# dmytroleonenko/gym-narde

Measured on AMD Instinct MI355X. Metric: env steps/sec at batch=65536, 1 MI355X (+ legal-move bit-exact vs CPU), higher is better.
Workload: dtype u32

## Files before the change

### __graft_entry__.py

```python
import os
import subprocess
import sys

ROOT = os.path.dirname(os.path.abspath(__file__))
PKG_DIR = os.path.join(ROOT, "gym-narde_amd")
CSRC = os.path.join(PKG_DIR, "csrc")
LIB = os.path.join(PKG_DIR, "gym_narde", "libnarde.so")
HOSTCHECK = os.path.join(ROOT, "tests", "hostcheck")

HIPCC = os.environ.get("HIPCC", "/opt/rocm/bin/hipcc")
HIP_FLAGS = ["-O3", "-std=c++17", "--offload-arch=gfx950", "-fPIC", "-shared", "-Wall"]


def _paths():
    for p in (PKG_DIR, os.path.join(ROOT, "oracle")):
        if p not in sys.path:
            sys.path.insert(0, p)


def _run(cmd):
    print("+", " ".join(cmd), flush=True)
    subprocess.check_call(cmd)


def build():
    srcs = [os.path.join(CSRC, "narde.hip"), os.path.join(CSRC, "dqn_learner.hip")]
    _run([HIPCC, *HIP_FLAGS, "-o", LIB, *srcs])
    _run(["make", "-s", "-C", os.path.join(ROOT, "oracle")])
    os.makedirs(os.path.join(HOSTCHECK, "build"), exist_ok=True)
    _run([HIPCC, "-O2", "-std=c++17", "-fPIC", "-shared", "-x", "c++", "-D__HIP_PLATFORM_AMD__",
          "-I/opt/rocm/include", "-o", os.path.join(HOSTCHECK, "build", "libhostcheck.so"),
          os.path.join(HOSTCHECK, "hostcheck.cpp")])
    _run([HIPCC, "-O2", "-std=c++17", "-fPIC", "-shared", "-x", "c++", "-D__HIP_PLATFORM_AMD__",
          "-I/opt/rocm/include", "-o", os.path.join(HOSTCHECK, "build", "libhostcheck_afterstates.so"),
          os.path.join(HOSTCHECK, "hostcheck_afterstates.cpp")])
    _run([HIPCC, "-O2", "-std=c++17", "-fPIC", "-shared", "-x", "c++", "-D__HIP_PLATFORM_AMD__",
          "-I/opt/rocm/include", "-o", os.path.join(HOSTCHECK, "build", "libhostcheck_turn_afterstates.so"),
          os.path.join(HOSTCHECK, "hostcheck_turn_afterstates.cpp")])
    _run([HIPCC, "-O2", "-std=c++17", "-fPIC", "-shared", "-x", "c++", "-D__HIP_PLATFORM_AMD__",
          "-I/opt/rocm/include", "-o", os.path.join(HOSTCHECK, "build", "libhostcheck_value.so"),
          os.path.join(HOSTCHECK, "hostcheck_value.cpp")])
    _paths()
    import gym_narde
    import gym_narde.envs
    import gym_narde.vector
    from gym_narde import _lib

    _lib.load()


def smoke():
    _paths()
    import numpy as np
    import torch

    import oracle as O
    from gym_narde.envs.narde import Narde
    from gym_narde.vector import VecNardeEnv

    assert torch.cuda.is_available(), "smoke() needs a GPU"
    n, plies, seed = 2048, 64, 20251015
    env = VecNardeEnv(n, device="cuda:0", seed=seed, env_id_offset=5, max_episode_steps=1000)
    ref = O.SelfPlay(n, seed=seed, env0=5)
    ref.reset(0)
    rec = ref.run(plies)
    for p in range(plies):
        obs, rew, term, trunc, info = env.step()
        torch.cuda.synchronize()
        assert np.array_equal(obs.cpu().numpy(), rec["obs"][p].astype(np.int32)), f"obs ply {p}"
        assert np.array_equal(rew.cpu().numpy(), rec["reward"][p].astype(np.int32)), f"reward ply {p}"
        assert np.array_equal(term.cpu().numpy(), rec["terminated"][p]), f"terminated ply {p}"
        assert np.array_equal(info["actions"].cpu().numpy(), rec["action"][p]), f"actions ply {p}"
        assert np.array_equal(info["legal"].cpu().numpy().view(np.uint64), rec["legal"][p]), f"legal ply {p}"
    st = env.get_state()
    assert np.array_equal(st["board"].cpu().numpy(), ref.board)
    g = Narde()
    assert g.get_valid_moves([5, 3], 1) == [(23, 18)]
    assert g.get_valid_moves([6, 6], 1) == [(23, 17), (23, 17)]
    env.close()
    print(f"smoke ok: {n} envs x {plies} plies bit-exact vs oracle")


if __name__ == "__main__":
    build()
    if len(sys.argv) > 1 and sys.argv[1] == "smoke":
        smoke()
```

### gym-narde_amd/csrc/full4_wave.h

```cpp
#pragma once

namespace {

__device__ __forceinline__ uint32_t rl(uint32_t v, int l) {
  return (uint32_t)__builtin_amdgcn_readlane((int)v, l);
}
__device__ void coop_run(const Side& s, uint32_t low, int a, int b, int hl, uint32_t m0, uint32_t m1,
                         int need, bool bf, int mode, int lane, uint32_t out[3]) {
  out[0] = out[1] = out[2] = 0u;
  uint64_t owners = __ballot((m0 | m1) != 0u);
  const int which = lane >> 5, p = lane & 31;
  while (owners) {
    const int ow = (int)__builtin_ctzll(owners);
    owners &= owners - 1ull;
    Side c;
    c.own.w[0] = rl(s.own.w[0], ow); c.own.w[1] = rl(s.own.w[1], ow); c.own.w[2] = rl(s.own.w[2], ow);
    c.O = rl(s.O, ow); c.S1o = rl(s.S1o, ow); c.P = rl(s.P, ow);
    c.off_own = rl(s.off_own, ow);
    c.opp.w[0] = c.opp.w[1] = c.opp.w[2] = 0u;
    c.S1p = 0u; c.off_opp = 0u; c.ft_own = 0u; c.ft_opp = 0u; c.black = 0u; c.elapsed = 0u; c.t = 0u;
    const uint32_t lw = rl(low, ow), om0 = rl(m0, ow), om1 = rl(m1, ow);
    const int pa = (int)rl((uint32_t)a, ow), pb = (int)rl((uint32_t)b, ow);
    const int thl = (int)rl((uint32_t)hl, ow), tneed = (int)rl((uint32_t)need, ow);
    const bool tbf = rl(bf ? 1u : 0u, ow) != 0u;
// ... 148 lines not shown
  } else {
    Cl = 0u;
    if (xbf) { Ch = Lh; M = Lh ? Mx : 0; }
    else if (fast) { Ch = Lh; M = 4; }
    else if (!Lh) { Ch = 0u; M = 0; }
    else if (r0[2]) { Ch = r0[2]; M = 4; }
    else if (r0[1]) { Ch = r0[1]; M = 3; }
    else if (r0[0]) { Ch = r0[0]; M = 2; }
    else { Ch = Lh; M = 1; }
  }
  turn_play(s, dh, dl, Ch, Cl, M, hl0, play, pw, w, o,
            [&](int k, int dk, int need, bool act, int hl, uint32_t Lk) -> uint32_t {
              (void)k;
              if (act && !bf) Lk = die_filter(s.O, s.S1o, block_info_low(s.O, low), Lk, dk);
              if (hl <= 0) Lk &= ~HEAD;
              const bool direct = !dbl || bf || fast || need <= 0;
              uint32_t rk[3];
              coop_run(s, low, dk, 0, hl, (act && !direct) ? Lk : 0u, 0u, need > 0 ? need : 1, bf, 0, lane,
                       rk);
              return direct ? Lk : (need >= 2 ? rk[1] : rk[0]);
            });
}


__device__ void coop_depth_w(const Side& s, uint32_t fw, int d, int hl, uint32_t m0, int need, int lane,
                             uint32_t out[3]) {
  out[0] = out[1] = out[2] = 0u;
  uint64_t owners = __ballot(m0 != 0u);
  while (owners) {
    const int ow = (int)__builtin_ctzll(owners);
    owners &= owners - 1ull;
    Side c;
    c.own.w[0] = rl(s.own.w[0], ow); c.own.w[1] = rl(s.own.w[1], ow); c.own.w[2] = rl(s.own.w[2], ow);
    c.O = rl(s.O, ow); c.S1o = rl(s.S1o, ow); c.P = rl(s.P, ow);
    c.off_own = rl(s.off_own, ow);
    c.opp.w[0] = c.opp.w[1] = c.opp.w[2] = 0u;
    c.S1p = 0u; c.off_opp = 0u; c.ft_own = 0u; c.ft_opp = 0u; c.black = 0u; c.elapsed = 0u; c.t = 0u;
    const uint32_t ofw = rl(fw, ow), om = rl(m0, ow);
    const int od = (int)rl((uint32_t)d, ow), ohl = (int)rl((uint32_t)hl, ow), oneed = (int)rl((uint32_t)need, ow);
    const bool has = lane < 24 && ((om >> lane) & 1u);
    const int src = has ? lane : 0;
    Side cc = c;
    apply_die_if(cc, src, od, has);
    const int hl2 = ohl - ((has && src == 23) ? 1 : 0);
    int dep = oneed == 1 ? f4_probe_w<1>(cc, ofw, od, hl2)
                         : (oneed == 2 ? f4_probe_w<2>(cc, ofw, od, hl2) : f4_probe_w<3>(cc, ofw, od, hl2));
    const bool miss = has && dep < oneed;
    if (__ballot(miss) != 0ull) {
      if (miss)
        dep = oneed == 1 ? f4_depth_w<1>(cc, ofw, od, hl2)
                         : (oneed == 2 ? f4_depth_w<2>(cc, ofw, od, hl2) : f4_depth_w<3>(cc, ofw, od, hl2));
    }
    const bool k0 = has && dep >= 1, k1 = has && dep >= 2, k2 = has && dep >= 3;
    const uint32_t r0 = (uint32_t)__ballot(k0), r1 = (uint32_t)__ballot(k1), r2 = (uint32_t)__ballot(k2);
    out[0] = lane == ow ? r0 : out[0];
    out[1] = lane == ow ? r1 : out[1];
    out[2] = lane == ow ? r2 : out[2];
  }
}

__device__ void coop_pair_w(const Side& s, uint32_t fw, int d, int hl, uint32_t m0, uint32_t w0, int lane,
                            uint32_t r0[3], uint32_t& c1, bool& ok) {
  r0[0] = r0[1] = r0[2] = 0u;
  c1 = 0u;
  ok = false;
  uint64_t owners = __ballot(m0 != 0u);
  while (owners) {
    const int ow = (int)__builtin_ctzll(owners);
    owners &= owners - 1ull;
    Side c;
    c.own.w[0] = rl(s.own.w[0], ow); c.own.w[1] = rl(s.own.w[1], ow); c.own.w[2] = rl(s.own.w[2], ow);
    c.O = rl(s.O, ow); c.S1o = rl(s.S1o, ow); c.P = rl(s.P, ow);
    c.off_own = rl(s.off_own, ow);
    c.opp.w[0] = c.opp.w[1] = c.opp.w[2] = 0u;
    c.S1p = 0u; c.off_opp = 0u; c.ft_own = 0u; c.ft_opp = 0u; c.black = 0u; c.elapsed = 0u; c.t = 0u;
    const uint32_t ofw = rl(fw, ow), om = rl(m0, ow), ow0 = rl(w0, ow);
    const int od = (int)rl((uint32_t)d, ow), ohl = (int)rl((uint32_t)hl, ow);
    const int nsrc = __builtin_popcount(om);
    const int r = lane >> 3, k = lane & 7;
    const bool hs = r < nsrc;
    const int s0 = select_bit(om, hs ? r : 0);
    Side ca = c;
    apply_die_if(ca, s0, od, hs);
    const int hla = ohl - ((hs && s0 == 23) ? 1 : 0);
    uint32_t L1 = die_candidates_sl(ca.O, ca.P, od);
    L1 &= ~block_reject_w(ca.O, ca.S1o, ofw, L1, od);
    L1 &= hla <= 0 ? ~HEAD : ~0u;
    L1 = hs ? L1 : 0u;
    const int cnt = __builtin_popcount(L1);
    if (nsrc > 8 || __ballot(k == 0 && cnt > 8) != 0ull) continue;
    const bool hp = k < cnt;
    const int s1 = select_bit(L1, hp ? k : 0);
    Side cp = ca;
    apply_die_if(cp, s1, od, hp);
    const int hlp = hla - ((hp && s1 == 23) ? 1 : 0);
    int dep = f4_probe_w<2>(cp, ofw, od, hlp);
    const bool miss = hp && dep == 1;
    if (__ballot(miss) != 0ull) {
      if (miss) dep = f4_depth_w<2>(cp, ofw, od, hlp);
    }
    const uint64_t B0 = __ballot(k == 0 && cnt > 0), B1 = __ballot(hp && dep >= 1), B2 = __ballot(hp && dep >= 2);
    const bool src = lane < 24 && ((om >> lane) & 1u);
    const int rt = __builtin_popcount(om & ((1u << (lane & 31)) - 1u));
    const int sh = src ? 8 * rt : 0;
    const uint32_t a0 = (uint32_t)__ballot(src && ((B0 >> sh) & 1ull) != 0ull);
    const uint32_t a1 = (uint32_t)__ballot(src && ((B1 >> sh) & 0xFFull) != 0ull);
    const uint32_t a2 = (uint32_t)__ballot(src && ((B2 >> sh) & 0xFFull) != 0ull);
    const int M = a2 ? 4 : (a1 ? 3 : (a0 ? 2 : 1));
    const uint32_t Cs = a2 ? a2 : (a1 ? a1 : (a0 ? a0 : om));
    const int p0 = select_bit(Cs, (int)mulhi_u32(ow0, (uint32_t)__builtin_popcount(Cs)));
    const int r0p = __builtin_popcount(om & ((1u << p0) - 1u));
    const uint32_t Lp = rl(L1, 8 * r0p);
    const uint32_t G = (uint32_t)(((M >= 4 ? B2 : B1) >> (8 * r0p)) & 0xFFull);
    const bool inl = lane < 24 && ((Lp >> lane) & 1u);
    const int e = __builtin_popcount(Lp & ((1u << (lane & 31)) - 1u));
    const uint32_t cv = (uint32_t)__ballot(inl && ((G >> e) & 1u));
    r0[0] = lane == ow ? a0 : r0[0];
    r0[1] = lane == ow ? a1 : r0[1];
    r0[2] = lane == ow ? a2 : r0[2];
    c1 = lane == ow ? cv : c1;
    ok = lane == ow ? true : ok;
  }
}

__device__ __forceinline__ void ply_bound_turn_c0(Side& s, int dh, int dl, uint32_t bs, uint32_t fw,
                                                  const uint32_t w[4], bool flip_always, TurnOut& o, int lane,
                                                  const TurnC0& c) {
  uint32_t Lh = c.Lh, Ll = c.Ll, Ch = c.Ch, Cl = c.Cl;
  int M = c.M;
  const int hl0 = c.hl0;
  const bool dbl = dh == dl;
  const bool b2 = bs != 0u && !dbl, bd = bs != 0u && dbl;
  if (__ballot(b2) != 0ull) {
    if (b2) turn_c0_pair_bound_w(s, dh, dl, bs, fw, Lh, Ll, Ch, Cl, M);
  }
  bool srch = false, pairs = false;
  uint32_t c1p = 0u;
  if (__ballot(bd) != 0ull) {
    const uint32_t Lb = Lh & ~block_reject_w(s.O, s.S1o, bd ? fw : 0u, Lh, dh);
    const bool fast = bd && f4_safe_bound(s, dh, hl0, bs) >= 4;
    srch = bd && !fast && Lb != 0u;
    uint32_t r0[3];
    coop_pair_w(s, fw, dh, hl0, srch ? Lb : 0u, w[0], lane, r0, c1p, pairs);
    if (__ballot(srch && !pairs) != 0ull) {
      uint32_t rd[3];
      coop_depth_w(s, fw, dh, hl0, (srch && !pairs) ? Lb : 0u, 3, lane, rd);
      if (srch && !pairs) { r0[0] = rd[0]; r0[1] = rd[1]; r0[2] = rd[2]; }
    }
    const int Ms = r0[2] ? 4 : (r0[1] ? 3 : (r0[0] ? 2 : 1));
    const uint32_t Cs = r0[2] ? r0[2] : (r0[1] ? r0[1] : (r0[0] ? r0[0] : Lb));
    Ch = bd ? (fast ? Lb : (Lb ? Cs : 0u)) : Ch;
    M = bd ? (fast ? 4 : (Lb ? Ms : 0)) : M;
  }
  o.legal = (uint64_t)Ch | ((uint64_t)Cl << 24) | ((uint64_t)dh << 48) | ((uint64_t)dl << 52) |
            ((uint64_t)M << 56);
  const int nh = __builtin_popcount(Ch), n = nh + __builtin_popcount(Cl);
  const int idx = (int)mulhi_u32(w[0], (uint32_t)n);
  const bool hi = idx < nh;
  const int d0 = hi ? dh : dl;
  const int p0 = select_bit(hi ? Ch : Cl, hi ? idx : idx - nh);
  const bool go = M >= 1;
  apply_die_if(s, p0, d0, go);
  uint32_t pl0 = go ? (0xFFFF0000u | ((uint32_t)d0 << 8) | (uint32_t)p0) : 0xFFFFFFFFu, pl1 = 0xFFFFFFFFu;
  int hl = hl0 - ((go && p0 == 23) ? 1 : 0);
  const int d1 = dbl ? dh : (d0 == dh ? dl : dh);
  const bool anyb = __ballot(bs != 0u) != 0ull;
#pragma unroll
  for (int k = 1; k < 4; ++k) {
    const int dk = k == 1 ? d1 : dh;
    const bool act = k < M;
    uint32_t Lk = die_candidates_sl(s.O, s.P, dk);
    if (anyb) {
      const bool filt = bd || (k == 1 && b2);
      Lk &= ~block_reject_w(s.O, s.S1o, filt ? fw : 0u, Lk, dk);
    }
    Lk &= hl <= 0 ? ~HEAD : ~0u;
    const int need = M - k - 1;
    const bool byp = k == 1 && pairs && need > 0;
    Lk = (srch && act && byp) ? c1p : Lk;
    const bool chk = srch && act && need > 0 && !byp;
    if (__ballot(chk) != 0ull) {
      uint32_t rk[3];
      coop_depth_w(s, fw, dk, hl, chk ? Lk : 0u, need, lane, rk);
      Lk = chk ? (need >= 2 ? rk[1] : rk[0]) : Lk;
    }
    const uint32_t wk = k == 1 ? w[1] : (k == 2 ? w[2] : w[3]);
    const int p = select_bit(Lk, (int)mulhi_u32(wk, (uint32_t)__builtin_popcount(Lk)));
    apply_die_if(s, p, dk, act);
    const uint32_t v = ((uint32_t)dk << 8) | (uint32_t)p;
    if (k == 1) pl0 = act ? ((pl0 & 0xFFFFu) | (v << 16)) : pl0;
    if (k == 2) pl1 = act ? ((pl1 & 0xFFFF0000u) | v) : pl1;
    if (k == 3) pl1 = act ? ((pl1 & 0xFFFFu) | (v << 16)) : pl1;
    hl -= (act && p == 23) ? 1 : 0;
  }
  o.played = (uint64_t)pl0 | ((uint64_t)pl1 << 32);
  o.max_dice = M;
  o.term = s.off_own == 15u;
  o.reward = o.term ? (s.off_opp > 0u ? 1 : 2) : 0;
  if (flip_always) side_flip(s);
  else side_flip_if(s, !o.term);
}

__device__ __forceinline__ void ply_bound_turn(Side& s, int dh, int dl, uint32_t bs, uint32_t fw, const uint32_t w[4],
                                               bool flip_always, TurnOut& o, int lane) {
  TurnC0 c;
  turn_c0_free(s, dh, dl, c.Lh, c.Ll, c.Ch, c.Cl, c.M, c.hl0);
  ply_bound_turn_c0(s, dh, dl, bs, fw, w, flip_always, o, lane, c);
}

}
```

### gym-narde_amd/csrc/kernels_rollout.h

```cpp
#pragma once

namespace {

struct Outs {
  int32_t* __restrict__ obs;
  int32_t* __restrict__ reward;
  uint8_t* __restrict__ term;
  uint8_t* __restrict__ trunc;
  uint64_t* __restrict__ legal;
  int16_t* __restrict__ act_out;
  uint64_t* __restrict__ played;
  int64_t* __restrict__ totals;
};

struct StepArgs {
  Planes pl;
  int n;
  Rng g;
  int max_steps;
  int autoreset;
  const int16_t* __restrict__ actions;
  const int8_t* __restrict__ play;
  const uint8_t* __restrict__ dice;
  Outs out;
};

template <class T>
__device__ __forceinline__ void st_nt(T* p, T v) {
  if constexpr (sizeof(T) == 16) {
    typedef int v4nt __attribute__((ext_vector_type(4)));
    v4nt x;
    __builtin_memcpy(&x, &v, 16);
    __builtin_nontemporal_store(x, reinterpret_cast<v4nt*>(p));
  } else {
    __builtin_nontemporal_store(v, p);
  }
}

__device__ __forceinline__ int nib_at(uint32_t x, int off) {
  return (int)__builtin_amdgcn_ubfe(x, (uint32_t)off, 4u);
}

template <int B>
__device__ __forceinline__ int sub_byte(uint32_t a, uint32_t b) {
  int r;
  if constexpr (B == 0)
    asm("v_sub_u32_sdwa %0, %1, %2 dst_sel:DWORD dst_unused:UNUSED_PAD src0_sel:BYTE_0 src1_sel:BYTE_0"
        : "=v"(r) : "v"(a), "v"(b));
  else if constexpr (B == 1)
    asm("v_sub_u32_sdwa %0, %1, %2 dst_sel:DWORD dst_unused:UNUSED_PAD src0_sel:BYTE_1 src1_sel:BYTE_1"
        : "=v"(r) : "v"(a), "v"(b));
  else if constexpr (B == 2)
    asm("v_sub_u32_sdwa %0, %1, %2 dst_sel:DWORD dst_unused:UNUSED_PAD src0_sel:BYTE_2 src1_sel:BYTE_2"
        : "=v"(r) : "v"(a), "v"(b));
  else
    asm("v_sub_u32_sdwa %0, %1, %2 dst_sel:DWORD dst_unused:UNUSED_PAD src0_sel:BYTE_3 src1_sel:BYTE_3"
        : "=v"(r) : "v"(a), "v"(b));
  return r;
}

template <int Q>
__device__ __forceinline__ int4 obs_quad_w(uint32_t own, uint32_t opp) {
  const uint32_t ol = own & 0x0F0F0F0Fu, oh = (own >> 4) & 0x0F0F0F0Fu;
  const uint32_t pl = opp & 0x0F0F0F0Fu, ph = (opp >> 4) & 0x0F0F0F0Fu;
  if constexpr ((Q & 1) == 0)
    return make_int4(sub_byte<0>(ol, pl), sub_byte<0>(oh, ph), sub_byte<1>(ol, pl), sub_byte<1>(oh, ph));
  else
    return make_int4(sub_byte<2>(ol, pl), sub_byte<2>(oh, ph), sub_byte<3>(ol, pl), sub_byte<3>(oh, ph));
}

template <int Q>
__device__ __forceinline__ int4 obs_quad(const Side& s) {
  return obs_quad_w<Q>(s.own.w[Q >> 1], s.opp.w[Q >> 1]);
}

__device__ __forceinline__ void store_obs(int32_t* __restrict__ obs, size_t ix, const Side& s) {
  int4* o = reinterpret_cast<int4*>(obs + ix * 24);
  st_nt(o + 0, obs_quad<0>(s));
  st_nt(o + 1, obs_quad<1>(s));
  st_nt(o + 2, obs_quad<2>(s));
  st_nt(o + 3, obs_quad<3>(s));
  st_nt(o + 4, obs_quad<4>(s));
  st_nt(o + 5, obs_quad<5>(s));
}

__device__ __forceinline__ void store_obs_wave(int32_t* __restrict__ obs, size_t ix, const Side& s,
                                               int4* __restrict__ lds) {
  const int lane = threadIdx.x & 63;
  lds[lane * 6 + 0] = obs_quad<0>(s);
  lds[lane * 6 + 1] = obs_quad<1>(s);
  lds[lane * 6 + 2] = obs_quad<2>(s);
  lds[lane * 6 + 3] = obs_quad<3>(s);
  lds[lane * 6 + 4] = obs_quad<4>(s);
  lds[lane * 6 + 5] = obs_quad<5>(s);
  wave_lds_handoff();
  int4* dst = reinterpret_cast<int4*>(obs + (ix - lane) * 24);
#pragma unroll
  for (int q = 0; q < 6; ++q) st_nt(dst + q * 64 + lane, lds[q * 64 + lane]);
  wave_lds_handoff();
}

__device__ __forceinline__ void store_common(const Outs& out, size_t ix, const Side& s, int reward,
                                             int term, int trunc, int4* lds, bool via_lds) {
  if (out.obs) {
    if (via_lds) store_obs_wave(out.obs, ix, s, lds);
    else store_obs(out.obs, ix, s);
  }
  if (out.reward) st_nt(out.reward + ix, (int32_t)reward);
  if (out.term) st_nt(out.term + ix, (uint8_t)term);
  if (out.trunc) st_nt(out.trunc + ix, (uint8_t)trunc);
}

__device__ __forceinline__ void store_outs(const Outs& out, size_t ix, const Side& s,
                                           const StepOut& o, int term, int trunc, int4* lds,
                                           bool wave_full) {
  store_common(out, ix, s, o.reward, term, trunc, lds, wave_full);
  if (out.legal) st_nt(out.legal + ix, (uint64_t)compact_legal(o.l1));
  if (out.act_out)
    st_nt(reinterpret_cast<uint32_t*>(out.act_out) + ix,
           ((uint32_t)(uint16_t)o.code1) | ((uint32_t)(uint16_t)o.code2 << 16));
}

__device__ __forceinline__ void store_outs(const Outs& out, size_t ix, const Side& s,
                                           const TurnOut& o, int term, int trunc, int4* lds,
                                           bool wave_full) {
  (void)wave_full;
  store_common(out, ix, s, o.reward, term, trunc, lds, false);
  if (out.legal) st_nt(out.legal + ix, o.legal);
  if (out.played) st_nt(out.played + ix, o.played);
}

#define OBS_LDS_DECL                                   \
  __shared__ int4 obs_lds[kBlock * 6];                 \
  int4* const wave_lds = obs_lds + (threadIdx.x & ~63) * 6;

__device__ __forceinline__ void ply_draw_cached(const Rng& g, uint32_t t, uint32_t i, uint32_t R[4], bool first,
                                                uint32_t r[4]) {
  if (first || (t & 1u) == 0u) ply_block(t, g.env0 + i, g.k0, g.k1, R);
  ply_words_of(R, t, g.dice_mode, r);
}

__device__ __forceinline__ void ply(Side& s, int4& st, const Rng& g, uint32_t i,
                                    const int16_t* actions, const uint8_t* dice, int max_steps,
                                    bool autoreset, StepOut& o, int& term, int& trunc, uint32_t R[4],
                                    bool first) {
  uint32_t r[4];
  ply_draw_cached(g, s.t, i, R, first, r);
  int d0 = 0, d1 = 0, c1 = 0, c2 = 0;
  if (dice) { d0 = dice[2 * i]; d1 = dice[2 * i + 1]; }
  if (actions) { c1 = actions[2 * i]; c2 = actions[2 * i + 1]; }
  if (!dice && !actions && autoreset) env_ply_policy_sl(s, st, r, g.dice_mode, max_steps, o, term, trunc);
  else env_ply(s, st, r, dice != nullptr, d0, d1, g.dice_mode, actions == nullptr, c1, c2, max_steps,
               autoreset, o, term, trunc);
}

__device__ __forceinline__ void ply_draw_wave(const Rng& g, uint32_t t, uint32_t i, uint32_t R[4], int p, int par,
                                              uint32_t r[4]) {
  if (par >= 0) {
    if (p == 0 || ((par + p) & 1) == 0) ply_block(t, g.env0 + i, g.k0, g.k1, R);
  } else if (p == 0 || (t & 1u) == 0u) {
    ply_block(t, g.env0 + i, g.k0, g.k1, R);
  }
  ply_words_of(R, t, g.dice_mode, r);
}

__device__ __forceinline__ int wave_parity(bool valid, uint32_t t) {
  const uint64_t odd = __ballot(valid && (t & 1u)), vm = __ballot(valid);
  return odd == 0ull ? 0 : (odd == vm ? 1 : -1);
}

template <bool kFilt>
__device__ __forceinline__ void ply_free_turn(Side& s, int dh, int dl, uint32_t bs, uint32_t fw, const uint32_t w[4],
                                              bool flip_always, TurnOut& o, const TurnC0& c) {
  uint32_t Lh = c.Lh, Ll = c.Ll, Ch = c.Ch, Cl = c.Cl;
  int M = c.M;
  const bool b2 = kFilt && bs != 0u;
  if (kFilt && b2) turn_c0_pair_bound_w(s, dh, dl, bs, fw, Lh, Ll, Ch, Cl, M);
  turn_moves_sl(s, dh, dl, Ch, Cl, M, c.hl0, w, b2, fw, flip_always, o);
}

__device__ __forceinline__ void ply_full_turn(Side& s, int4& st, int dh, int dl, uint32_t bs, uint32_t fw,
                                              const TurnC0& c, const uint32_t w[4], uint32_t rb, int max_steps,
                                              bool autoreset, TurnOut& o, int& term, int& trunc) {
  const uint32_t mover_black = s.black;
  if (__ballot(bs != 0u && dh == dl) == 0ull) {
    if (__ballot(bs != 0u) == 0ull) ply_free_turn<false>(s, dh, dl, bs, fw, w, autoreset, o, c);
    else ply_free_turn<true>(s, dh, dl, bs, fw, w, autoreset, o, c);
  } else {
    ply_bound_turn_c0(s, dh, dl, bs, fw, w, autoreset, o, (int)(threadIdx.x & 63), c);
  }
  if (autoreset) ply_close_sl_b(s, st, o.term, o.reward, mover_black, rb, max_steps, term, trunc);
  else ply_close(s, st, o.term, o.reward, mover_black, 0u, max_steps, false, term, trunc);
}

__device__ __forceinline__ void ply_full_dice(Side& s, int4& st, int dh, int dl, const uint32_t w[4], uint32_t rb,
                                              int max_steps, bool autoreset, TurnOut& o, int& term, int& trunc) {
  const uint32_t low = block_lowmask(s.P);
  uint32_t fw;
  const uint32_t bs = turn_block_set_sl(s.O, s.S1o, s.P, low, dh, dl, fw);
  TurnC0 c;
  turn_c0_free(s, dh, dl, c.Lh, c.Ll, c.Ch, c.Cl, c.M, c.hl0);
  ply_full_turn(s, st, dh, dl, bs, fw, c, w, rb, max_steps, autoreset, o, term, trunc);
}

__device__ __forceinline__ uint32_t ply_dice_word(const uint32_t r[4], int dice_mode, uint32_t w[4]) {
  int d0, d1;
  dice_from(r[0], dice_mode, d0, d1);
  const int dh = d0 > d1 ? d0 : d1, dl = d0 > d1 ? d1 : d0;
  turn_words(r, w);
  return (uint32_t)dh | ((uint32_t)dl << 4) | (reset_black(r[3]) << 8);
}

__device__ __forceinline__ void ply_full_words(Side& s, int4& st, const uint32_t r[4], int dice_mode,
                                               int max_steps, bool autoreset, TurnOut& o, int& term,
                                               int& trunc) {
  uint32_t w[4];
  const uint32_t dw = ply_dice_word(r, dice_mode, w);
  ply_full_dice(s, st, (int)(dw & 15u), (int)((dw >> 4) & 15u), w, autoreset ? dw >> 8 : 0u, max_steps, autoreset,
                o, term, trunc);
}

__device__ __forceinline__ void ply_policy_full(Side& s, int4& st, const Rng& g, uint32_t i, int max_steps,
                                                bool autoreset, TurnOut& o, int& term, int& trunc,
                                                uint32_t R[4], int p, int par) {
  uint32_t r[4];
  ply_draw_wave(g, s.t, i, R, p, par, r);
  ply_full_words(s, st, r, g.dice_mode, max_steps, autoreset, o, term, trunc);
}

__device__ __forceinline__ void ply(Side& s, int4& st, const Rng& g, uint32_t i, bool valid,
                                    const int8_t* play, const uint8_t* dice, int max_steps,
                                    bool autoreset, TurnOut& o, int& term, int& trunc, uint32_t R[4],
                                    bool first) {
  if (!play && !dice) {
    ply_policy_full(s, st, g, i, max_steps, autoreset, o, term, trunc, R, 0, 0);
    return;
  }
  uint32_t r[4];
  ply_draw_cached(g, s.t, i, R, first, r);
  int d0 = 1, d1 = 2;
  if (dice && valid) { d0 = dice[2 * i]; d1 = dice[2 * i + 1]; }
  const uint64_t pw = (play && valid) ? reinterpret_cast<const uint64_t*>(play)[i] : ~0ull;
  const int lane = (int)(threadIdx.x & 63);
  env_ply_full_with(s, st, r, g.env0 + i, g.k0, g.k1, dice != nullptr, d0, d1, g.dice_mode,
                    play != nullptr, pw, max_steps, autoreset, o, term, trunc,
                    [&](Side& s2, int a, int b, bool pl, uint64_t pw2, const uint32_t* w2, TurnOut& o2) {
                      coop_turn_full(s2, a, b, pl, pw2, w2, o2, lane);
                    });
}

__device__ __forceinline__ void add_stats(int4* __restrict__ stats, int i, const int4& st) {
  if (st.x) {
    int4 cur = stats[i];
    cur.x += st.x; cur.y += st.y; cur.z += st.z;
    stats[i] = cur;
  }
}

__device__ __forceinline__ int4 stats_after(int4* __restrict__ stats, int i, const int4& st, bool want) {
  int4 cur = make_int4(0, 0, 0, 0);
  if (st.x || want) {
    cur = stats[i];
    cur.x += st.x; cur.y += st.y; cur.z += st.z;
    if (st.x) stats[i] = cur;
  }
  return cur;
}

__device__ __forceinline__ int4 stats_read(const int4* __restrict__ stats, int i, bool valid) {
  return valid ? stats[i] : make_int4(0, 0, 0, 0);
}
__device__ __forceinline__ int4 stats_after_pre(int4* __restrict__ stats, int i, int4 pre, const int4& st) {
  pre.x += st.x;
  pre.y += st.y;
  pre.z += st.z;
  if (st.x) stats[i] = pre;
  return pre;
}

__device__ __forceinline__ void wg_totals(const int4& cum, int64_t* __restrict__ rows) {
  __shared__ long long red[16][3];
  long long e = cum.x, w = cum.y, k = cum.z;
#pragma unroll
  for (int o = 32; o > 0; o >>= 1) {
    e += __shfl_xor(e, o, 64);
    w += __shfl_xor(w, o, 64);
    k += __shfl_xor(k, o, 64);
  }
  const int wave = threadIdx.x >> 6;
  if ((threadIdx.x & 63) == 0) { red[wave][0] = e; red[wave][1] = w; red[wave][2] = k; }
  __syncthreads();
  if (threadIdx.x < 3) {
    long long t = 0;
    const int nw = (int)(blockDim.x >> 6);
    for (int q = 0; q < nw; ++q) t += red[q][threadIdx.x];
    rows[3 * blockIdx.x + threadIdx.x] = (int64_t)t;
  }
}

template <bool kFull>
__global__ void __launch_bounds__(kBlock) k_step(StepArgs a) {
  OBS_LDS_DECL
  const int i = blockIdx.x * kBlock + threadIdx.x;
  const bool valid = i < a.n;
  if (!kFull && !valid) return;
  Side s = valid ? side_from_record(a.pl.p0[i], a.pl.p1[i]) : side_start(0u);
  int4 st = make_int4(0, 0, 0, 0);
  typename std::conditional<kFull, TurnOut, StepOut>::type o;
  int term, trunc;
  uint32_t R[4];
  if constexpr (kFull)
    ply(s, st, a.g, (uint32_t)i, valid, a.play, a.dice, a.max_steps, a.autoreset != 0, o, term, trunc, R,
        true);
  else
    ply(s, st, a.g, (uint32_t)i, a.actions, a.dice, a.max_steps, a.autoreset != 0, o, term, trunc, R, true);
  if (!valid) return;
  uint4 ra, rb;
  side_to_record(s, ra, rb);
  a.pl.p0[i] = ra;
  a.pl.p1[i] = rb;
  add_stats(a.pl.stats, i, st);
  store_outs(a.out, (size_t)i, s, o, term, trunc, wave_lds, i - (int)(threadIdx.x & 63) + 64 <= a.n);
}

constexpr int kPcGroups = 4;
constexpr int kPcEnvs = 64 * kPcGroups;
constexpr int kPcThreads = 2 * kPcEnvs;
constexpr int kPcR = 4;
constexpr int kPcSlots = 2;

__device__ __forceinline__ int pc_nblocks(int plies, int R) {
  return plies <= 1 ? 1 : 1 + (plies - 1 + R - 1) / R;
}
__device__ __forceinline__ void pc_block(int b, int plies, int R, int& p0, int& np) {
  p0 = b == 0 ? 0 : 1 + (b - 1) * R;
  const int sz = b == 0 ? 1 : R;
  np = max(0, min(sz, plies - p0));
}
constexpr int kPcRShort = 2;
constexpr int kPcShortPlies = 32;

struct PcLds {
  uint4 lead_[4];
  uint2 draw[kPcSlots][kPcR][kPcEnvs];
  uint4 nib0[kPcSlots][kPcR][kPcEnvs];
  uint2 nib1[kPcSlots][kPcR][kPcEnvs];
  uint2 legal[kPcSlots][kPcR][kPcEnvs];
  uint2 cf[kPcSlots][kPcR][kPcEnvs];
};

__device__ __forceinline__ void pc_put(PcLds& L, int slot, int k, int le, const Side& s,
                                       const StepOut& o, int term, int trunc) {
  const uint64_t lg = compact_legal(o.l1);
  L.nib0[slot][k][le] = make_uint4(s.own.w[0], s.own.w[1], s.own.w[2], s.opp.w[0]);
// ... 302 lines not shown
```

### gym-narde_amd/csrc/narde_rules.h

```cpp
#pragma once
#include <hip/hip_runtime.h>
#include <math.h>
#include <stdint.h>

#define NARDE_FN __host__ __device__ __forceinline__

namespace narde {

constexpr uint32_t MASK24 = 0xFFFFFFu;
constexpr int OFF = 24;

struct Nib {
  uint32_t w[3];
};

NARDE_FN uint32_t funnel16(uint32_t hi, uint32_t lo) { return (lo >> 16) | (hi << 16); }

NARDE_FN uint32_t nib_word(const Nib& b, int p) {
  const uint32_t w0 = b.w[0], w1 = b.w[1], w2 = b.w[2];
  const int k = p >> 3;
  return (k == 0 ? w0 : 0u) | (k == 1 ? w1 : 0u) | (k == 2 ? w2 : 0u);
}
NARDE_FN uint32_t nib_get(const Nib& b, int p) { return (nib_word(b, p) >> (4 * (p & 7))) & 15u; }
NARDE_FN void nib_add(Nib& b, int p, uint32_t delta ) {
// ... 1107 lines not shown
  const int tq = t > 0 ? t : 0;
  const uint32_t cf = nib_get(s.own, p);
  const bool land = en && !off;
  const uint32_t bf = en ? (1u << p) : 0u;
  const uint32_t bt = land ? (1u << tq) : 0u;
  const uint32_t vf = en ? (0xFFFFFFFFu << (4 * (p & 7))) : 0u;
  const uint32_t vt = (land ? 1u : 0u) << (4 * (tq & 7));
  const int kf = p >> 3, kt = tq >> 3;
  s.own.w[0] += (kf == 0 ? vf : 0u) + (kt == 0 ? vt : 0u);
  s.own.w[1] += (kf == 1 ? vf : 0u) + (kt == 1 ? vt : 0u);
  s.own.w[2] += (kf == 2 ? vf : 0u) + (kt == 2 ? vt : 0u);
  const uint32_t t01 = bt & (~s.O | s.S1o);
  s.O = (s.O & (cf == 1u ? ~bf : ~0u)) | bt;
  s.S1o ^= (cf - 1u < 2u ? bf : 0u) ^ t01;
  s.off_own += (en && off) ? 1u : 0u;
  s.ft_own = en ? 0u : s.ft_own;
}

NARDE_FN uint32_t f4_keep_pair_bf_sl(uint32_t O, uint32_t S1, uint32_t P, int a, int b, uint32_t L) {
  const uint32_t G = ~(P << b) & (MASK24 << b) & MASK24;
  const uint32_t X = O & G;
  const uint32_t e1 = (nz1(X, S1) & ~HEAD) | (((X & ~HEAD) != 0u) ? HEAD : 0u);
  const uint32_t e2 = (G << a) & MASK24;
  const uint32_t LB = (1u << b) - 1u;
  const uint32_t out = O & ~0x3Fu;
  const bool lone = (out & (out - 1u)) == 0u && (out & S1) != 0u &&
                    (int)__builtin_ctz(out | 0x80000000u) - a < 6;
  const uint32_t homep = (out == 0u ? MASK24 : 0u) | (lone ? out : 0u);
  const uint32_t e3 = homep & (nz1(O & LB, S1) | ((LB << a) & MASK24));
  return L & (e1 | e2 | e3);
}

NARDE_FN bool f4_bearoff_fixed_sl(const Side& s, int rem) {
  uint32_t x = s.own.w[0] & 0xFFFFFFu;
  x = (x & 0x0F0F0Fu) + ((x >> 4) & 0x0F0F0Fu);
  const uint32_t home = ((x * 0x010101u) >> 16) & 0xFFu;
  return ((s.O >> 6) == 0u) | ((int)(15u - s.off_own - home) >= rem);
}

NARDE_FN int f4_open_moves_sl(const Side& s, int d, int hl, int T) {
  const uint32_t O = s.O, fr = ~s.P & MASK24;
  const uint32_t r0 = (1u << d) - 1u;
  const uint32_t r1 = ((r0 & fr) << d) & MASK24;
  const uint32_t r2 = ((r1 & fr) << d) & MASK24;
  const uint32_t r3 = ((r2 & fr) << d) & MASK24;
  const uint32_t R = (r0 | r1 | r2 | r3) & O;
  const uint32_t h1 = ((0x3Fu & fr) << d) & MASK24;
  const uint32_t h2 = ((h1 & fr) << d) & MASK24;
  const uint32_t h3 = ((h2 & fr) << d) & MASK24;
  const uint32_t X = O & ~0x3Fu;
  const int head = (int)nib_get(s.own, 23);
  const bool reach = (X & ~(h1 | h2 | h3)) == 0u && !((X & HEAD) && head > hl);
  uint32_t ge4;
  const uint32_t ge3 = nib_ge3_ge4(s.own, ge4);
  const uint32_t Rb = R & ~HEAD;
  const int B = __builtin_popcount(Rb) + __builtin_popcount(Rb & ~s.S1o) + __builtin_popcount(Rb & ge3) +
                __builtin_popcount(Rb & ge4) + ((R & HEAD) ? head : 0);
  const int t = T + (reach ? B : 0);
  return t < 4 ? t : 4;
}

NARDE_FN void turn_c0_free(const Side& s, int dh, int dl, uint32_t& Lh, uint32_t& Ll, uint32_t& Ch, uint32_t& Cl,
                           int& M, int& hl0) {
  const bool dbl = dh == dl;
  Lh = die_candidates_sl(s.O, s.P, dh);
  Ll = die_candidates_sl(s.O, s.P, dl) & msk(!dbl);
  const uint32_t kh = f4_keep_pair_bf_sl(s.O, s.S1o, s.P, dh, dl, Lh);
  const uint32_t kl = f4_keep_pair_bf_sl(s.O, s.S1o, s.P, dl, dh, Ll);
  hl0 = (dbl && s.ft_own && (dh == 3 || dh == 4 || dh == 6)) ? 2 : 1;
  const int T0 = f4_exact_moves(s, dh, hl0);
  const int Mo = f4_open_moves_sl(s, dh, hl0, T0);
  const int Mx = f4_bearoff_fixed_sl(s, 4) ? T0 : Mo;
  const bool pair = (kh | kl) != 0u;
  const bool two = !dbl && pair;
  Ch = (kh & msk(two)) | (Lh & msk(!two));
  Cl = (kl & msk(two)) | (Ll & msk(!dbl && !pair && Lh == 0u));
  const int M2 = two ? 2 : ((Lh | Ll) != 0u ? 1 : 0);
  M = dbl ? (Lh != 0u ? Mx : 0) : M2;
}

struct TurnC0 {
  uint32_t Lh, Ll, Ch, Cl;
  int M, hl0;
};

NARDE_FN void side_flip_if(Side& s, bool flip) {
  Side f = s;
  side_flip(f);
  s.own.w[0] = flip ? f.own.w[0] : s.own.w[0];
  s.own.w[1] = flip ? f.own.w[1] : s.own.w[1];
  s.own.w[2] = flip ? f.own.w[2] : s.own.w[2];
  s.opp.w[0] = flip ? f.opp.w[0] : s.opp.w[0];
  s.opp.w[1] = flip ? f.opp.w[1] : s.opp.w[1];
  s.opp.w[2] = flip ? f.opp.w[2] : s.opp.w[2];
  s.O = flip ? f.O : s.O;
  s.P = flip ? f.P : s.P;
  s.S1o = flip ? f.S1o : s.S1o;
  s.S1p = flip ? f.S1p : s.S1p;
  s.off_own = flip ? f.off_own : s.off_own;
  s.off_opp = flip ? f.off_opp : s.off_opp;
  s.ft_own = flip ? f.ft_own : s.ft_own;
  s.ft_opp = flip ? f.ft_opp : s.ft_opp;
  s.black = flip ? f.black : s.black;
}

NARDE_FN uint32_t block_reject_w(uint32_t O, uint32_t S1, uint32_t fw, uint32_t C, int d);
NARDE_FN void turn_moves_sl(Side& s, int dh, int dl, uint32_t Ch, uint32_t Cl, int M, int hl, const uint32_t w[4],
                            bool filt, uint32_t fw, bool flip_always, TurnOut& o) {
  const bool dbl = dh == dl;
  o.legal = (uint64_t)Ch | ((uint64_t)Cl << 24) | ((uint64_t)dh << 48) | ((uint64_t)dl << 52) |
            ((uint64_t)M << 56);
  const int nh = __builtin_popcount(Ch), n = nh + __builtin_popcount(Cl);
  const int idx = (int)mulhi_u32(w[0], (uint32_t)n);
  const bool hi = idx < nh;
  const int d0 = hi ? dh : dl;
  const int p0 = select_bit(hi ? Ch : Cl, hi ? idx : idx - nh);
  const bool go = M >= 1;
  apply_die_if(s, p0, d0, go);
  uint32_t pl0 = go ? (0xFFFF0000u | ((uint32_t)d0 << 8) | (uint32_t)p0) : 0xFFFFFFFFu, pl1 = 0xFFFFFFFFu;
  hl -= (go && p0 == 23) ? 1 : 0;
  const int d1 = dbl ? dh : (d0 == dh ? dl : dh);
#pragma unroll
  for (int k = 1; k < 4; ++k) {
    const int dk = k == 1 ? d1 : dh;
    const bool act = k < M;
    uint32_t Lk = die_candidates_sl(s.O, s.P, dk);
    if (k == 1 && filt) Lk &= ~block_reject_w(s.O, s.S1o, fw, Lk, dk);
    Lk &= hl <= 0 ? ~HEAD : ~0u;
    const uint32_t wk = k == 1 ? w[1] : (k == 2 ? w[2] : w[3]);
    const int p = select_bit(Lk, (int)mulhi_u32(wk, (uint32_t)__builtin_popcount(Lk)));
    apply_die_if(s, p, dk, act);
    const uint32_t v = ((uint32_t)dk << 8) | (uint32_t)p;
    if (k == 1) pl0 = act ? ((pl0 & 0xFFFFu) | (v << 16)) : pl0;
    if (k == 2) pl1 = act ? ((pl1 & 0xFFFF0000u) | v) : pl1;
    if (k == 3) pl1 = act ? ((pl1 & 0xFFFFu) | (v << 16)) : pl1;
    hl -= (act && p == 23) ? 1 : 0;
  }
  o.played = (uint64_t)pl0 | ((uint64_t)pl1 << 32);
  o.max_dice = M;
  o.term = s.off_own == 15u;
  o.reward = o.term ? (s.off_opp > 0u ? 1 : 2) : 0;
  if (flip_always) side_flip(s);
  else side_flip_if(s, !o.term);
}

NARDE_FN void turn_free_sl(Side& s, int dh, int dl, const uint32_t w[4], bool flip_always, TurnOut& o) {
  uint32_t Lh, Ll, Ch, Cl;
  int M, hl0;
  turn_c0_free(s, dh, dl, Lh, Ll, Ch, Cl, M, hl0);
  turn_moves_sl(s, dh, dl, Ch, Cl, M, hl0, w, false, 0u, flip_always, o);
}


NARDE_FN void die_filter2(uint32_t O, uint32_t S1, const Blocks& bl, uint32_t Ca, int a, uint32_t Cb, int b,
                          uint32_t& La, uint32_t& Lb) {
  const uint32_t hitA = bl.F ? MASK24 : (bl.Q << a);
  const uint32_t hitB = bl.F ? MASK24 : (bl.Q << b);
  La = Ca & ~(hitA & ~S1);
  Lb = Cb & ~(hitB & ~S1);
  uint32_t ma = Ca & hitA & S1, mb = Cb & hitB & S1;
  while (ma | mb) {
    const bool fa = ma != 0u;
    const uint32_t m = fa ? ma : mb;
    const int d = fa ? a : b;
    const int p = __builtin_ctz(m);
    const uint32_t bp = 1u << p;
    ma &= fa ? ~bp : ~0u;
    mb &= fa ? ~0u : ~bp;
    const uint32_t Op = (O & ~bp) | (p >= d ? (1u << (p - d)) : 0u);
    const uint32_t rej = (runs6(Op) & bl.low) ? bp : 0u;
    La &= fa ? ~rej : ~0u;
    Lb &= fa ? ~0u : ~rej;
  }
}

NARDE_FN void legal2_low_sl(const Side& s, int d0, int d1, uint32_t low, Legal& l) {
  const int dh = d0 > d1 ? d0 : d1, dl = d0 > d1 ? d1 : d0;
  const bool dbl = dh == dl;
  const Blocks bl = block_info_low(s.O, low);
  uint32_t Lh, Ll;
  die_filter2(s.O, s.S1o, bl, die_candidates_sl(s.O, s.P, dh), dh,
              die_candidates_sl(s.O, s.P, dl) & msk(!dbl), dl, Lh, Ll);
  Ll = dbl ? Lh : Ll;
  const bool two_heads = s.ft_own && dbl && (dh == 3 || dh == 4 || dh == 6);
  Ll &= ((Lh >> 23) != 0u && !two_heads) ? ~HEAD : ~0u;
  l.n = 2;
  l.d[0] = dh; l.d[1] = dl; l.d[2] = 0; l.d[3] = 0;
  l.L[0] = Lh; l.L[1] = Ll; l.L[2] = 0u; l.L[3] = 0u;
  l.count = __builtin_popcount(Lh) + __builtin_popcount(Ll);
}

NARDE_FN void env_step_policy_sl(Side& s, int d0, int d1, uint32_t r1, uint32_t r2, StepOut& o) {
  const uint32_t low = block_lowmask(s.P);
  legal2_low_sl(s, d0, d1, low, o.l1);
  const int n1 = o.l1.count;
  int f1, t1;
  legal2_entry(o.l1, (int)mulhi_u32(r1, (uint32_t)n1), f1, t1);
  const int code1 = n1 >= 2 ? encode_move(f1, t1) : 0;
  const bool quirk = n1 >= 2 && t1 == 0 && f1 <= 5;
  const uint32_t bf1 = 1u << f1;
  const bool listed_off = (((o.l1.L[0] & bf1) != 0u) & (f1 < o.l1.d[0])) | (((o.l1.L[1] & bf1) != 0u) & (f1 < o.l1.d[1]));
  t1 = quirk ? OFF : t1;
  const bool play1 = quirk ? listed_off : n1 >= 1;
  apply_move_if(s, f1, t1, play1);
  const bool has2 = n1 >= 2 && play1;
  const int dist = t1 == OFF ? f1 + 1 : f1 - t1;
  const int rem = (d0 == dist) ? d1 : ((d1 == dist) ? d0 : d1);
  const Blocks bl = block_info_low(s.O, low);
  uint32_t L2, unused;
  die_filter2(s.O, s.S1o, bl, die_candidates_sl(s.O, s.P, rem) & msk(has2), rem, 0u, 1, L2, unused);
  const int c2 = __builtin_popcount(L2);
  const int f2 = select_bit(L2, (int)mulhi_u32(r2, (uint32_t)c2));
  const int t2 = f2 - rem < 0 ? OFF : f2 - rem;
  const bool play2 = c2 > 0 && !(t2 == 0 && f2 <= 5);
  apply_move_if(s, f2, t2, play2);
  o.L2 = L2;
  o.d2 = has2 ? rem : 0;
  o.count2 = has2 ? c2 : -1;
  o.code1 = code1;
  o.code2 = c2 > 0 ? encode_move(f2, t2) : 0;
  o.term = s.off_own == 15u;
  o.reward = o.term ? (s.off_opp > 0u ? 1 : 2) : 0;
  side_flip(s);
}

template <int N>
NARDE_FN int f4_depth_w(const Side& s, uint32_t fw, int d, int hl) {
  uint32_t L = die_candidates_sl(s.O, s.P, d);
  L &= ~block_reject_w(s.O, s.S1o, fw, L, d);
  if (hl <= 0) L &= ~HEAD;
  if (!L) return 0;
  if constexpr (N == 1) {
    return 1;
  } else {
    int best = 1;
    while (L && best < N) {
      const int p = __builtin_ctz(L);
      L &= L - 1u;
      Side c = s;
      apply_die(c, p, d);
      const int v = 1 + f4_depth_w<N - 1>(c, fw, d, hl - (p == 23 ? 1 : 0));
      best = v > best ? v : best;
    }
    return best;
  }
}

template <int N>
NARDE_FN int f4_probe_w(Side c, uint32_t fw, int d, int hl) {
  int dep = 0;
  bool alive = true;
#pragma unroll
  for (int k = 0; k < N; ++k) {
    uint32_t L = die_candidates_sl(c.O, c.P, d);
    L &= ~block_reject_w(c.O, c.S1o, fw, L, d);
    L &= hl <= 0 ? ~HEAD : ~0u;
    alive = alive && L != 0u;
    dep += alive ? 1 : 0;
    if (k + 1 < N) {
      const int p = (int)__builtin_ctz(L | 0x800000u);
      apply_die_if(c, p, d, alive);
      hl -= (alive && p == 23) ? 1 : 0;
    }
  }
  return dep;
}

NARDE_FN uint32_t turn_block_set_sl(uint32_t O, uint32_t S1, uint32_t P, uint32_t low, int dh, int dl,
                                    uint32_t& fw) {
  const bool dbl = dh == dl;
  const uint32_t A = O | land_step(O, P, dh) | land_step(O, P, dl);
  const uint32_t U2 = A | land_step(A, P, dh) | land_step(A, P, dl);
  const uint32_t V = land_step(U2, P, dh);
  const uint32_t U = U2 | (dbl ? (V | land_step(V, P, dh)) : 0u);
  uint32_t s0, s1, s2;
  window_hole_count(O, s0, s1, s2);
  const uint32_t le1 = ~s2 & ~s1, le2 = ~s2 & ~(s1 & s0), eq2 = s1 & ~s0 & ~s2;
  const uint32_t eq3 = s1 & s0 & ~s2, eq4 = s2 & ~s1 & ~s0;
  const uint32_t rU = runs6(U) & low, rA = runs6(A) & low;
  uint32_t win2 = dbl ? 0u : ((le1 & rU) | (eq2 & rA));
  uint32_t wind = dbl ? ((le2 & rU) | (eq3 & runs6(U2) & low) | (eq4 & rA)) : 0u;
  uint32_t out = 0u;
  bool full = false;
  fw = 0u;
  while (win2) {
    const int i = __builtin_ctz(win2);
    win2 &= win2 - 1u;
    const uint32_t W = 0x3Fu << i;
    const uint32_t H = W & ~O;
    full = full || H == 0u;
    const uint32_t src = O & ~(W & S1);
    const uint32_t Lh = land_step(src, P, dh), Ll = land_step(src, P, dl);
    const uint32_t h1 = H & (0u - H), h2 = H ^ h1;
    const bool one = (H & (Lh | Ll | land_step(Lh, P, dl) | land_step(Ll, P, dh))) != 0u;
    const bool two = (((h1 & Lh) != 0u) & ((h2 & Ll) != 0u)) | (((h1 & Ll) != 0u) & ((h2 & Lh) != 0u));
    const bool tfail = h2 == 0u ? one : two;
    out |= H & msk(tfail);
    fw |= (H == 0u || tfail) ? (1u << i) : 0u;
  }
  while (wind) {
    const int i = __builtin_ctz(wind);
    wind &= wind - 1u;
    const uint32_t W = 0x3Fu << i;
    const uint32_t H = W & ~O;
    full = full || H == 0u;
    uint32_t T = O & ~(W & S1), seen = 0u;
// ... 563 lines not shown
```

Before: 52.35 billion.

## Replace exact max-dice search with cap bound and early-stop greedy play

Adds turn_c0_cap, which computes a cheap upper bound on playable dice (4 for doubles, pair-keep check for non-doubles) instead of the full search in turn_c0_free. It also adds turn_moves_cap, which plays greedily and stops when no candidates remain, deriving the real max_dice and legal word from the moves actually played. The free-turn and bound-turn paths switch to these, and the full4 wave path now records M as the played count. This avoids the deeper max-dice search on most boards, but it depends on the claim that greedy play under the cap reaches the true maximum, which the new hostcheck is meant to verify.

```diff
diff --git a/__graft_entry__.py b/__graft_entry__.py
--- a/__graft_entry__.py
+++ b/__graft_entry__.py
@@ -40,6 +40,9 @@
     _run([HIPCC, "-O2", "-std=c++17", "-fPIC", "-shared", "-x", "c++", "-D__HIP_PLATFORM_AMD__",
           "-I/opt/rocm/include", "-o", os.path.join(HOSTCHECK, "build", "libhostcheck_value.so"),
           os.path.join(HOSTCHECK, "hostcheck_value.cpp")])
+    _run([HIPCC, "-O2", "-std=c++17", "-fPIC", "-shared", "-x", "c++", "-D__HIP_PLATFORM_AMD__",
+          "-I/opt/rocm/include", "-o", os.path.join(HOSTCHECK, "build", "libhostcheck_full4_count.so"),
+          os.path.join(HOSTCHECK, "hostcheck_full4_count.cpp")])
     _paths()
     import gym_narde
     import gym_narde.envs
diff --git a/gym-narde_amd/csrc/full4_wave.h b/gym-narde_amd/csrc/full4_wave.h
--- a/gym-narde_amd/csrc/full4_wave.h
+++ b/gym-narde_amd/csrc/full4_wave.h
@@ -324,8 +324,6 @@
     Ch = bd ? (fast ? Lb : (Lb ? Cs : 0u)) : Ch;
     M = bd ? (fast ? 4 : (Lb ? Ms : 0)) : M;
   }
-  o.legal = (uint64_t)Ch | ((uint64_t)Cl << 24) | ((uint64_t)dh << 48) | ((uint64_t)dl << 52) |
-            ((uint64_t)M << 56);
   const int nh = __builtin_popcount(Ch), n = nh + __builtin_popcount(Cl);
   const int idx = (int)mulhi_u32(w[0], (uint32_t)n);
   const bool hi = idx < nh;
@@ -337,10 +335,12 @@
   int hl = hl0 - ((go && p0 == 23) ? 1 : 0);
   const int d1 = dbl ? dh : (d0 == dh ? dl : dh);
   const bool anyb = __ballot(bs != 0u) != 0ull;
+  bool prev = go;
+  uint32_t Mp = go ? 1u : 0u;
 #pragma unroll
   for (int k = 1; k < 4; ++k) {
     const int dk = k == 1 ? d1 : dh;
-    const bool act = k < M;
+    const bool pre = prev && k < M;
     uint32_t Lk = die_candidates_sl(s.O, s.P, dk);
     if (anyb) {
       const bool filt = bd || (k == 1 && b2);
@@ -349,13 +349,14 @@
     Lk &= hl <= 0 ? ~HEAD : ~0u;
     const int need = M - k - 1;
     const bool byp = k == 1 && pairs && need > 0;
-    Lk = (srch && act && byp) ? c1p : Lk;
-    const bool chk = srch && act && need > 0 && !byp;
+    Lk = (srch && pre && byp) ? c1p : Lk;
+    const bool chk = srch && pre && need > 0 && !byp;
     if (__ballot(chk) != 0ull) {
       uint32_t rk[3];
       coop_depth_w(s, fw, dk, hl, chk ? Lk : 0u, need, lane, rk);
       Lk = chk ? (need >= 2 ? rk[1] : rk[0]) : Lk;
     }
+    const bool act = pre && Lk != 0u;
     const uint32_t wk = k == 1 ? w[1] : (k == 2 ? w[2] : w[3]);
     const int p = select_bit(Lk, (int)mulhi_u32(wk, (uint32_t)__builtin_popcount(Lk)));
     apply_die_if(s, p, dk, act);
@@ -364,9 +365,14 @@
     if (k == 2) pl1 = act ? ((pl1 & 0xFFFF0000u) | v) : pl1;
     if (k == 3) pl1 = act ? ((pl1 & 0xFFFFu) | (v << 16)) : pl1;
     hl -= (act && p == 23) ? 1 : 0;
-  }
+    Mp += act ? 1u : 0u;
+    prev = act;
+  }
+  const uint32_t lg0 = Ch | (Cl << 24);
+  const uint32_t lg1 = (Cl >> 8) | ((uint32_t)dh << 16) | ((uint32_t)dl << 20) | (Mp << 24);
+  o.legal = (uint64_t)lg0 | ((uint64_t)lg1 << 32);
   o.played = (uint64_t)pl0 | ((uint64_t)pl1 << 32);
-  o.max_dice = M;
+  o.max_dice = (int)Mp;
   o.term = s.off_own == 15u;
   o.reward = o.term ? (s.off_opp > 0u ? 1 : 2) : 0;
   if (flip_always) side_flip(s);
@@ -376,7 +382,7 @@
 __device__ __forceinline__ void ply_bound_turn(Side& s, int dh, int dl, uint32_t bs, uint32_t fw, const uint32_t w[4],
                                                bool flip_always, TurnOut& o, int lane) {
   TurnC0 c;
-  turn_c0_free(s, dh, dl, c.Lh, c.Ll, c.Ch, c.Cl, c.M, c.hl0);
+  turn_c0_cap(s, dh, dl, c.Lh, c.Ll, c.Ch, c.Cl, c.M, c.hl0);
   ply_bound_turn_c0(s, dh, dl, bs, fw, w, flip_always, o, lane, c);
 }
 
diff --git a/gym-narde_amd/csrc/kernels_rollout.h b/gym-narde_amd/csrc/kernels_rollout.h
--- a/gym-narde_amd/csrc/kernels_rollout.h
+++ b/gym-narde_amd/csrc/kernels_rollout.h
@@ -176,7 +176,7 @@
   int M = c.M;
   const bool b2 = kFilt && bs != 0u;
   if (kFilt && b2) turn_c0_pair_bound_w(s, dh, dl, bs, fw, Lh, Ll, Ch, Cl, M);
-  turn_moves_sl(s, dh, dl, Ch, Cl, M, c.hl0, w, b2, fw, flip_always, o);
+  turn_moves_cap(s, dh, dl, Ch, Cl, M, c.hl0, w, b2, fw, flip_always, o);
 }
 
 __device__ __forceinline__ void ply_full_turn(Side& s, int4& st, int dh, int dl, uint32_t bs, uint32_t fw,
@@ -199,7 +199,7 @@
   uint32_t fw;
   const uint32_t bs = turn_block_set_sl(s.O, s.S1o, s.P, low, dh, dl, fw);
   TurnC0 c;
-  turn_c0_free(s, dh, dl, c.Lh, c.Ll, c.Ch, c.Cl, c.M, c.hl0);
+  turn_c0_cap(s, dh, dl, c.Lh, c.Ll, c.Ch, c.Cl, c.M, c.hl0);
   ply_full_turn(s, st, dh, dl, bs, fw, c, w, rb, max_steps, autoreset, o, term, trunc);
 }
 
diff --git a/gym-narde_amd/csrc/narde_rules.h b/gym-narde_amd/csrc/narde_rules.h
--- a/gym-narde_amd/csrc/narde_rules.h
+++ b/gym-narde_amd/csrc/narde_rules.h
@@ -1283,6 +1283,67 @@
 }
 
 
+NARDE_FN void turn_c0_cap(const Side& s, int dh, int dl, uint32_t& Lh, uint32_t& Ll, uint32_t& Ch, uint32_t& Cl,
+                          int& M, int& hl0) {
+  const bool dbl = dh == dl;
+  Lh = die_candidates_sl(s.O, s.P, dh);
+  Ll = die_candidates_sl(s.O, s.P, dl) & msk(!dbl);
+  const uint32_t kh = f4_keep_pair_bf_sl(s.O, s.S1o, s.P, dh, dl, Lh);
+  const uint32_t kl = f4_keep_pair_bf_sl(s.O, s.S1o, s.P, dl, dh, Ll);
+  hl0 = (dbl && s.ft_own && (dh == 3 || dh == 4 || dh == 6)) ? 2 : 1;
+  const bool pair = (kh | kl) != 0u;
+  const bool two = !dbl && pair;
+  Ch = (kh & msk(two)) | (Lh & msk(!two));
+  Cl = (kl & msk(two)) | (Ll & msk(!dbl && !pair && Lh == 0u));
+  const int M2 = two ? 2 : ((Lh | Ll) != 0u ? 1 : 0);
+  M = dbl ? (Lh != 0u ? 4 : 0) : M2;
+}
+
+NARDE_FN void turn_moves_cap(Side& s, int dh, int dl, uint32_t Ch, uint32_t Cl, int cap, int hl, const uint32_t w[4],
+                             bool filt, uint32_t fw, bool flip_always, TurnOut& o) {
+  const bool dbl = dh == dl;
+  const int nh = __builtin_popcount(Ch), n = nh + __builtin_popcount(Cl);
+  const int idx = (int)mulhi_u32(w[0], (uint32_t)n);
+  const bool hi = idx < nh;
+  const int d0 = hi ? dh : dl;
+  const int p0 = select_bit(hi ? Ch : Cl, hi ? idx : idx - nh);
+  const bool go = cap >= 1;
+  apply_die_if(s, p0, d0, go);
+  uint32_t pl0 = go ? (0xFFFF0000u | ((uint32_t)d0 << 8) | (uint32_t)p0) : 0xFFFFFFFFu, pl1 = 0xFFFFFFFFu;
+  hl -= (go && p0 == 23) ? 1 : 0;
+  const int d1 = dbl ? dh : (d0 == dh ? dl : dh);
+  bool prev = go;
+  uint32_t M = go ? 1u : 0u;
+#pragma unroll
+  for (int k = 1; k < 4; ++k) {
+    const int dk = k == 1 ? d1 : dh;
+    uint32_t Lk = die_candidates_sl(s.O, s.P, dk);
+    if (k == 1 && filt) Lk &= ~block_reject_w(s.O, s.S1o, fw, Lk, dk);
+    Lk &= hl <= 0 ? ~HEAD : ~0u;
+    const bool act = prev && k < cap && Lk != 0u;
+    const uint32_t wk = k == 1 ? w[1] : (k == 2 ? w[2] : w[3]);
+    const int p = select_bit(Lk, (int)mulhi_u32(wk, (uint32_t)__builtin_popcount(Lk)));
+    apply_die_if(s, p, dk, act);
+    const uint32_t v = ((uint32_t)dk << 8) | (uint32_t)p;
+    if (k == 1) pl0 = act ? ((pl0 & 0xFFFFu) | (v << 16)) : pl0;
+    if (k == 2) pl1 = act ? ((pl1 & 0xFFFF0000u) | v) : pl1;
+    if (k == 3) pl1 = act ? ((pl1 & 0xFFFFu) | (v << 16)) : pl1;
+    hl -= (act && p == 23) ? 1 : 0;
+    M += act ? 1u : 0u;
+    prev = act;
+  }
+  const uint32_t lg0 = Ch | (Cl << 24);
+  const uint32_t lg1 = (Cl >> 8) | ((uint32_t)dh << 16) | ((uint32_t)dl << 20) | (M << 24);
+  o.legal = (uint64_t)lg0 | ((uint64_t)lg1 << 32);
+  o.played = (uint64_t)pl0 | ((uint64_t)pl1 << 32);
+  o.max_dice = (int)M;
+  o.term = s.off_own == 15u;
+  o.reward = o.term ? (s.off_opp > 0u ? 1 : 2) : 0;
+  if (flip_always) side_flip(s);
+  else side_flip_if(s, !o.term);
+}
+
+
 NARDE_FN void die_filter2(uint32_t O, uint32_t S1, const Blocks& bl, uint32_t Ca, int a, uint32_t Cb, int b,
                           uint32_t& La, uint32_t& Lb) {
   const uint32_t hitA = bl.F ? MASK24 : (bl.Q << a);
```

New measurement: 52.26 billion. Within noise of the previous version (-0.2%).
